# vikasdimaniya/video-fingerprinting

Hardware: AMD Instinct MI355X
Metric: 1080p frames/sec embed+detect (higher is better)
Workload: dtype f32

## Files before the change

### video-fingerprinting_amd/csrc/offmark_kernels.hip

```cpp
#include <hip/hip_runtime.h>
#include <hip/hip_ext.h>

#include <atomic>
#include <cstdint>
#include <cstdio>
#include <cstring>
#include <type_traits>

#include "../../include/offmark_hip.h"

#include "common.hiph"
#include "readout.hiph"
#include "dct_kernels.hiph"
#include "svd_kernels.hiph"
#include "svd8_kernels.hiph"
#include "misc_kernels.hiph"
#include "planar_kernels.hiph"
#include "svd_planar_kernels.hiph"
#include "copies_kernels.hiph"
#include "planar_copies_kernels.hiph"
#include "resync_kernels.hiph"
#include "dct_resync_kernels.hiph"
#include "planar_resync_kernels.hiph"

// ... 77 lines not shown
    const unsigned grid = (unsigned)(vec < 256 * 2048 ? (vec + 255) / 256 : 2048);
    hipLaunchKernelGGL(zero_kernel, dim3(grid), dim3(256), 0, s, static_cast<uint8_t *>(p), bytes);
    return hipGetLastError();
}

constexpr int kMaxChunk = 65535;

template <class Body>
int for_chunks(int n, int cap, Body &&body) {
    for (int f0 = 0; f0 < n; f0 += cap)
        if (int rc = body(f0, n - f0 < cap ? n - f0 : cap)) return rc;
    return OFMK_OK;
}

template <class F>
void with_bool(bool b, F &&f) {
    if (b) f(std::true_type{});
    else f(std::false_type{});
}
template <class F>
void with_fmt(int layout, F &&f) {
    if (layout == OFMK_YUV_I420) f(std::integral_constant<int, FMT_I420>{});
    else f(std::integral_constant<int, FMT_NV12>{});
}
template <class F>
void with_svd_mode(int mode, bool multi, F &&f) {
    if (mode == SVD_DETECT) f(std::integral_constant<int, SVD_DETECT>{}, std::false_type{});
    else if (mode == SVD_DETECT_SOFT) f(std::integral_constant<int, SVD_DETECT_SOFT>{}, std::false_type{});
    else if (mode == SVD_EMBED) with_bool(multi, [&](auto mu) { f(std::integral_constant<int, SVD_EMBED>{}, mu); });
    else with_bool(multi, [&](auto mu) { f(std::integral_constant<int, SVD_EMBED_VERIFY>{}, mu); });
}

struct Workspace {
    float *rec;
    float *delta;
    unsigned long long *ysum;
    unsigned long long *ysum2;
    int frames;
    int tiles;
    size_t plane;
};

constexpr size_t kFixedBytes = 4096;

size_t tiles_per_frame(int H, int W) { return ((size_t)(H / 8) * (W / 8) + kThreads - 1) / kThreads; }

size_t per_frame_bytes(int H, int W) {
    const size_t nblk = (size_t)(H / 8) * (W / 8);
    return nblk * (kRec + 1) * sizeof(float) + 2 * tiles_per_frame(H, W) * 8;
}

int carve(void *ws, size_t bytes, int H, int W, int want_frames, Workspace &out) {
    if (!ws) return fail(OFMK_E_ARG, "workspace is null%s");
    if ((uintptr_t)ws % 256) return fail(OFMK_E_ARG, "workspace must be 256-byte aligned%s");
    const size_t per = per_frame_bytes(H, W);
    if (bytes < per + kFixedBytes) return fail(OFMK_E_WORKSPACE, "workspace smaller than ofmk_workspace_bytes(1, H, W)%s");
    size_t cap = (bytes - kFixedBytes) / per;
    if (want_frames > 0 && (size_t)want_frames < cap) cap = want_frames;
    if (cap > (size_t)kMaxChunk) cap = kMaxChunk;
    const size_t nblk = (size_t)(H / 8) * (W / 8);
    char *p = static_cast<char *>(ws);
    out.frames = (int)cap;
    out.tiles = (int)tiles_per_frame(H, W);
    out.plane = cap * nblk;
    out.rec = reinterpret_cast<float *>(p);
    p += align256(out.plane * kRec * sizeof(float));
    out.delta = reinterpret_cast<float *>(p);
    p += align256(out.plane * sizeof(float));
    out.ysum = reinterpret_cast<unsigned long long *>(p);
    p += align256(cap * out.tiles * 8);
    out.ysum2 = reinterpret_cast<unsigned long long *>(p);
    return OFMK_OK;
}

int check_opts(const ofmk_opts *o) {
    if (o && ((o->flags & ~(uint32_t)(OFMK_F_SEPARATE_DETECT | OFMK_F_LINEAR_TILES | OFMK_F_XCD_TILES | OFMK_F_PARTIAL_COUNTS)) || o->xcds > 64u))
        return fail(OFMK_E_ARG, "ofmk_opts: unknown flag bits or xcds > 64%s");
    if (o && (o->flags & OFMK_F_LINEAR_TILES) && (o->flags & OFMK_F_XCD_TILES))
        return fail(OFMK_E_ARG, "ofmk_opts: OFMK_F_LINEAR_TILES and OFMK_F_XCD_TILES exclude each other%s");
    return OFMK_OK;
}

int check_dims(int n, int H, int W) {
    if (n <= 0) return fail(OFMK_E_ARG, "n must be positive%s");
    if (H < 8 || W < 8) return fail(OFMK_E_ARG, "H and W must be at least 8%s");
    if ((long long)H * W >= (1LL << 28)) return fail(OFMK_E_ARG, "frame too large (H*W must be < 2^28)%s");
    return OFMK_OK;
}

int check_embed_args(const void *in, const void *out, int n, int H, int W, const uint8_t *wm, int n_wm) {
    int rc = check_dims(n, H, W);
    if (rc) return rc;
    if (!in || !out || !wm) return fail(OFMK_E_ARG, "null frame or watermark pointer%s");
    if (n_wm < 1) return fail(OFMK_E_ARG, "n_wm must be >= 1%s");
    return OFMK_OK;
}

int check_detect_args(const void *in, int n, int H, int W, int L, const int32_t *counts, const uint8_t *bits) {
    int rc = check_dims(n, H, W);
    if (rc) return rc;
    if (!in) return fail(OFMK_E_ARG, "null frame pointer%s");
    if (L < 1) return fail(OFMK_E_ARG, "payload length L must be >= 1%s");
    if (!counts && !bits) return fail(OFMK_E_ARG, "both outputs (counts, bits) are null%s");
    return OFMK_OK;
}

int check_soft_args(const void *in, int n, int H, int W, int L, const long long *soft) {
    if (int rc = check_dims(n, H, W)) return rc;
    if (!in || !soft) return fail(OFMK_E_ARG, "null pointer%s");
    if (L < 1) return fail(OFMK_E_ARG, "payload length L must be >= 1%s");
    return OFMK_OK;
}

Geom make_geom(int H, int W, const Workspace &ws, int frames = 0, int xcds = 0) {
    Geom g;
    g.frames = frames;
    g.xcds = xcds;
    g.W = W;
    g.wb = W / 8;
    g.inv_wb = 1.0f / (float)g.wb;
    g.nblk = (H / 8) * (W / 8);
    g.frame_stride = (size_t)H * W * 3;
    g.plane = ws.plane;
    return g;
}

dim3 grid_2d(int units_per_frame, int n) { return dim3((unsigned)((units_per_frame + kThreads - 1) / kThreads), (unsigned)n); }

dim3 xcd_grid(int blocks_per_frame, int n, int xcds = 0) {
    const unsigned tiles = (unsigned)((blocks_per_frame + kThreads - 1) / kThreads);
    const unsigned long long G = (unsigned long long)tiles * (unsigned)n;
    const unsigned long long X = xcds > 1 ? (unsigned long long)xcds : 1ull;
    return dim3((unsigned)(((G + X - 1) / X) * X));
}

bool aligned_rows(const void *p, int W, size_t elem) {
    const size_t need = elem == 1 ? 8 : 16;
    return W % 8 == 0 && (uintptr_t)p % need == 0;
}

void launch_copy_fringe(const uint8_t *in, uint8_t *out, int n, int H, int W, int Hc, int Wc, hipStream_t s) {
    const size_t fringe = (size_t)(H - Hc) * W * 3 + (size_t)Hc * (W - Wc) * 3;
    if (fringe == 0) return;
    const unsigned gx = (unsigned)((fringe + 256 * 4 - 1) / (256 * 4));
    for_chunks(n, kMaxChunk, [&](int f0, int cf) {
        const size_t fo = (size_t)f0 * H * W * 3;
        hipLaunchKernelGGL(copy_fringe_kernel, dim3(gx < 1024 ? gx : 1024, (unsigned)cf), dim3(256), 0, s, in + fo, out + fo, H, W, Hc, Wc);
        return OFMK_OK;
    });
}

int launch_copy_fringe_copies(const uint8_t *in, uint8_t *out, int copies, int n, int H, int W, hipStream_t s) {
    if (H % 8 == 0 && W % 8 == 0) return OFMK_OK;
    for (int q = 0; q < copies; ++q) launch_copy_fringe(in, out + (size_t)q * n * H * W * 3, n, H, W, (H / 8) * 8, (W / 8) * 8, s);
    HIP_TRY(hipGetLastError());
    return OFMK_OK;
}

int launch_analyze(const void *frames, int src, int n, int H, int W, const Workspace &ws, const Ctx &cx,
                   int32_t *zero_counts = nullptr, int L = 0) {
    hipStream_t s = cx.s;
    const Geom g = make_geom(H, W, ws, n);
    const dim3 grid = xcd_grid(g.nblk, n);
    ScopedTiming timing(KIND_ANALYZE, cx);
    constexpr unsigned kAnalyzeLdsCap = 48u * 1024u;
    with_bool(aligned_rows(frames, W, src == SRC_RGB8 ? 1 : 4), [&](auto al) {
        constexpr bool AL = decltype(al)::value;
        if (src == SRC_RGB8) OFMK_TIMED_LAUNCH(timing, (analyze_kernel<SRC_RGB8, AL>), grid, dim3(kThreads), kAnalyzeLdsCap, s, frames, g, ws.rec, ws.ysum, zero_counts, L);
        else OFMK_TIMED_LAUNCH(timing, (analyze_kernel<SRC_YUV32F, AL>), grid, dim3(kThreads), 0, s, frames, g, ws.rec, ws.ysum, zero_counts, L);
    });
    HIP_TRY(hipGetLastError());
    return OFMK_OK;
}

int launch_finalize(FinArgs a, int n, const Ctx &cx) {
    const int per_wg = kThreads * kFinItems;
    const dim3 grid((unsigned)((a.N + per_wg - 1) / per_wg), (unsigned)n);
    ScopedTiming timing(KIND_FINALIZE, cx);
    with_bool(a.delta || a.soft || a.y_dc || a.lum || a.tex || a.step || a.c21_pre || a.c21_post, [&](auto full) {
        OFMK_TIMED_LAUNCH(timing, finalize_kernel<decltype(full)::value>, grid, dim3(kThreads), 0, cx.s, a);
    });
    HIP_TRY(hipGetLastError());
    return OFMK_OK;
}

MarkArgs mark_args(const Workspace &ws, int H, int W, const uint8_t *wm, int n_wm, const int32_t *wm_row, double alpha) {
    MarkArgs m;
    m.rec = ws.rec;
    m.ysum = ws.ysum;
    m.wm = wm;
    m.wm_row = wm_row;
    m.n_wm = n_wm;
    m.N = (int)((long long)H * W / 64);
    m.alpha = alpha;
    return m;
}

int launch_mark_rgb8(const uint8_t *in, uint8_t *out, int n, int H, int W, const uint8_t *wm, int n_wm, const int32_t *wm_row,
                     double alpha, const Workspace &ws, bool fused, const Ctx &cx) {
    hipStream_t s = cx.s;
    const int xc = tile_xcds(cx, (size_t)n * H * W * 3);
    const Geom g = make_geom(H, W, ws, n, xc);
    const dim3 grid = xcd_grid(g.nblk, n, xc);
    const MarkArgs m = mark_args(ws, H, W, wm, n_wm, wm_row, alpha);
    {
        ScopedTiming timing(fused ? KIND_MARK_FUSED : KIND_MARK, cx);
        with_bool(aligned_rows(in, W, 1) && aligned_rows(out, W, 1), [&](auto al) {
            constexpr bool AL = decltype(al)::value;
            if (fused) OFMK_TIMED_LAUNCH(timing, (mark_rgb8_kernel<AL, true>), grid, dim3(kThreads), 0, s, in, out, g, m, ws.rec, ws.ysum2);
            else if (xc > 1) OFMK_TIMED_LAUNCH(timing, (mark_rgb8_kernel<AL, false, true>), grid, dim3(kThreads), 0, s, in, out, g, m, ws.rec, ws.ysum2);
            else OFMK_TIMED_LAUNCH(timing, (mark_rgb8_kernel<AL, false>), grid, dim3(kThreads), 0, s, in, out, g, m, ws.rec, ws.ysum2);
        });
    }
    HIP_TRY(hipGetLastError());
    if (in != out && (H % 8 || W % 8)) {
        launch_copy_fringe(in, out, n, H, W, (H / 8) * 8, (W / 8) * 8, s);
        HIP_TRY(hipGetLastError());
    }
    return OFMK_OK;
}

struct RecView {
    const float *rec;
    const unsigned long long *ysum;
    size_t plane;
    int tiles;
};
RecView input_records(const Workspace &ws) { return {ws.rec, ws.ysum, ws.plane, ws.tiles}; }
RecView marked_records(const Workspace &ws) { return {ws.rec, ws.ysum2, ws.plane, ws.tiles}; }

FinArgs fin_base(const RecView &v, int H, int W, double alpha) {
    FinArgs a;
    memset(&a, 0, sizeof(a));
    a.rec = v.rec;
    a.plane = v.plane;
    a.ysum = v.ysum;
    a.tiles = v.tiles;
    a.nblk = (H / 8) * (W / 8);
    a.N = (int)((long long)H * W / 64);
    a.L = 1;
    a.n_wm = 1;
    a.alpha = alpha;
    return a;
}

int launch_mark_yuv32f(float *yuv, int n, int H, int W, const uint8_t *wm, int n_wm, const int32_t *wm_row, double alpha,
                       const Workspace &ws, const Ctx &cx) {
    FinArgs a = fin_base(input_records(ws), H, W, alpha);
    a.wm = wm;
    a.wm_row = wm_row;
    a.n_wm = n_wm;
    a.delta = ws.delta;
    if (int rc = launch_finalize(a, n, cx)) return rc;
    const Geom g = make_geom(H, W, ws);
    hipLaunchKernelGGL(mark_yuv32f_kernel, grid_2d(g.nblk, n), dim3(kThreads), 0, cx.s, yuv, g, ws.delta);
    HIP_TRY(hipGetLastError());
    return OFMK_OK;
}

int launch_payloads(const int32_t *counts, int n, int L, int n_bits, const int32_t *perm, uint8_t *payload, hipStream_t s) {
    hipLaunchKernelGGL(degenerate_kernel, dim3((unsigned)n), dim3(kThreads), 0, s, counts, L, n_bits, perm, payload);
    HIP_TRY(hipGetLastError());
    return OFMK_OK;
}

CopyArgs make_copy_args(int copies, int n, int f0, const int32_t *wm_rows, size_t frame_bytes, size_t counts_per_frame = 0,
                        size_t bits_per_frame = 0) {
    CopyArgs k;
    memset(&k, 0, sizeof(k));
    k.copies = copies;
    k.rows_stride = n;
    k.wm_rows = wm_rows ? wm_rows + f0 : nullptr;
    k.out_stride = (size_t)n * frame_bytes;
    k.counts_stride = (size_t)n * counts_per_frame;
    k.bits_stride = (size_t)n * bits_per_frame;
    return k;
}

int launch_mark_copies_rgb8(const uint8_t *in, uint8_t *out, int copies, int n, int f0, int cf, int H, int W, const uint8_t *wm,
                            int n_wm, const int32_t *wm_rows, double alpha, const Workspace &ws, const Ctx &cx) {
    const size_t fs = (size_t)H * W * 3;
    const uint8_t *pin = in + (size_t)f0 * fs;
    uint8_t *pout = out + (size_t)f0 * fs;
    const int xc = tile_xcds(cx, (size_t)cf * fs);
    const Geom g = make_geom(H, W, ws, cf, xc);
    const dim3 grid = xcd_grid(g.nblk, cf, xc);
    const MarkArgs m = mark_args(ws, H, W, wm, n_wm, nullptr, alpha);
    const CopyArgs k = make_copy_args(copies, n, f0, wm_rows, fs);
    ScopedTiming timing(KIND_MARK, cx);
    with_bool(aligned_rows(in, W, 1) && aligned_rows(out, W, 1), [&](auto al) {
        OFMK_TIMED_LAUNCH(timing, mark_copies_rgb8_kernel<decltype(al)::value>, grid, dim3(kThreads), 0, cx.s, pin, pout, g, m, k);
    });
    HIP_TRY(hipGetLastError());
    return OFMK_OK;
}

struct CopiesWorkspace {
    Workspace base;
    float *rec;
    unsigned long long *ysum;
    size_t plane;
};

size_t per_frame_copies_bytes(int copies, int H, int W) {
    const size_t nblk = (size_t)(H / 8) * (W / 8);
    return per_frame_bytes(H, W) + (size_t)copies * (nblk * kRec * sizeof(float) + tiles_per_frame(H, W) * 8);
}

int carve_copies(void *ws, size_t bytes, int copies, int H, int W, int want_frames, CopiesWorkspace &out) {
    if (!ws) return fail(OFMK_E_ARG, "workspace is null%s");
    if ((uintptr_t)ws % 256) return fail(OFMK_E_ARG, "workspace must be 256-byte aligned%s");
    const size_t per = per_frame_copies_bytes(copies, H, W);
    if (bytes < per + kFixedBytes) return fail(OFMK_E_WORKSPACE, "workspace smaller than ofmk_copies_workspace_bytes(1, copies, H, W)%s");
    size_t cap = (bytes - kFixedBytes) / per;
    if (want_frames > 0 && (size_t)want_frames < cap) cap = want_frames;
    if (cap > (size_t)kMaxChunk) cap = kMaxChunk;
    if (int rc = carve(ws, bytes, H, W, (int)cap, out.base)) return rc;
    const size_t nblk = (size_t)(H / 8) * (W / 8);
    char *p = reinterpret_cast<char *>(out.base.ysum2) + align256(cap * out.base.tiles * 8);
    out.plane = (size_t)copies * cap * nblk;
    out.rec = reinterpret_cast<float *>(p);
    p += align256(out.plane * kRec * sizeof(float));
    out.ysum = reinterpret_cast<unsigned long long *>(p);
    return OFMK_OK;
}

RecView copy_records(const CopiesWorkspace &ws, int q, int nblk) {
    return {ws.rec + (size_t)q * ws.base.frames * nblk, ws.ysum + (size_t)q * ws.base.frames * ws.base.tiles, ws.plane, ws.base.tiles};
}

int launch_mark_verify_copies_rgb8(const uint8_t *in, uint8_t *out, int copies, int n, int f0, int cf, int H, int W, const uint8_t *wm,
                                   int n_wm, const int32_t *wm_rows, double alpha, int L, const CopyRecs &v, const Workspace &ws,
                                   const Ctx &cx) {
    const size_t fs = (size_t)H * W * 3;
    const uint8_t *pin = in + (size_t)f0 * fs;
    uint8_t *pout = out + (size_t)f0 * fs;
    const int xc = tile_xcds(cx, (size_t)cf * fs);
    const Geom g = make_geom(H, W, ws, cf, xc);
    const dim3 grid = xcd_grid(g.nblk, cf, xc);
    const MarkArgs m = mark_args(ws, H, W, wm, n_wm, nullptr, alpha);
    const CopyArgs k = make_copy_args(copies, n, f0, wm_rows, fs, (size_t)L, (size_t)m.N);
    ScopedTiming timing(KIND_MARK_FUSED, cx);
    with_bool(aligned_rows(in, W, 1) && aligned_rows(out, W, 1), [&](auto al) {
        OFMK_TIMED_LAUNCH(timing, mark_verify_copies_rgb8_kernel<decltype(al)::value>, grid, dim3(kThreads), 0, cx.s, pin, pout, g, m, k, v);
    });
    HIP_TRY(hipGetLastError());
    return OFMK_OK;
}

int check_planar(int layout, int H, int W, const void *a, const void *b) {
    if (layout != OFMK_YUV_I420 && layout != OFMK_YUV_NV12) return fail(OFMK_E_ARG, "layout must be OFMK_YUV_I420 or OFMK_YUV_NV12%s");
    if (H % 8 || W % 8) return fail(OFMK_E_ARG, "planar 4:2:0 entry points need H and W to be multiples of 8%s");
    if ((a && (uintptr_t)a % 8) || (b && (uintptr_t)b % 8)) return fail(OFMK_E_ARG, "planar frame buffers must be 8-byte aligned%s");
    return OFMK_OK;
}

PGeom make_pgeom(int layout, int H, int W, size_t plane) {
    PGeom g;
    g.W = W;
    g.wb = W / 8;
    g.inv_wb = 1.0f / (float)g.wb;
    g.nblk = (H / 8) * (W / 8);
    g.frame_stride = (size_t)H * W * 3 / 2;
    g.u_off = (size_t)H * W;
    g.v_off = layout == OFMK_YUV_I420 ? g.u_off + (size_t)H * W / 4 : g.u_off + 1;
    g.cpitch = layout == OFMK_YUV_I420 ? W / 2 : W;
    g.plane = plane;
    return g;
}

int launch_analyze_yuv420(const uint8_t *frames, int layout, int n, int H, int W, const Workspace &ws, const Ctx &cx,
                          int32_t *zero_counts = nullptr, int L = 0) {
    const PGeom g = make_pgeom(layout, H, W, ws.plane);
    ScopedTiming timing(KIND_PLANAR_ANALYZE, cx);
    with_fmt(layout, [&](auto fmt) {
        OFMK_TIMED_LAUNCH(timing, analyze_yuv420_kernel<decltype(fmt)::value>, grid_2d(g.nblk, n), dim3(kThreads), 0, cx.s, frames, g, ws.rec, ws.ysum, zero_counts, L);
    });
    HIP_TRY(hipGetLastError());
    return OFMK_OK;
}

int launch_mark_yuv420(const uint8_t *in, uint8_t *out, int layout, int n, int H, int W, const uint8_t *wm, int n_wm, const int32_t *wm_row,
                       double alpha, const Workspace &ws, bool fused, const Ctx &cx) {
    const PGeom g = make_pgeom(layout, H, W, ws.plane);
    const MarkArgs m = mark_args(ws, H, W, wm, n_wm, wm_row, alpha);
    ScopedTiming timing(KIND_PLANAR_MARK, cx);
    with_fmt(layout, [&](auto fmt) { with_bool(fused, [&](auto fu) {
        OFMK_TIMED_LAUNCH(timing, (mark_yuv420_kernel<decltype(fmt)::value, decltype(fu)::value>), grid_2d(g.nblk, n), dim3(kThreads), 0, cx.s, in, out, g, m, ws.rec, ws.ysum2);
    }); });
    HIP_TRY(hipGetLastError());
    return OFMK_OK;
}

int convert_yuv420(uint8_t *yuv, uint8_t *rgb, bool to_rgb, int layout, int n, int H, int W, void *stream, const ofmk_opts *opts) {
    if (int orc = check_opts(opts)) return orc;
    int rc = check_dims(n, H, W);
    if (rc) return rc;
    if (!yuv || !rgb) return fail(OFMK_E_ARG, "null pointer%s");
    if ((rc = check_planar(layout, H, W, yuv, rgb))) return rc;
    const PGeom g = make_pgeom(layout, H, W, 0);
    hipStream_t s = static_cast<hipStream_t>(stream);
    for_chunks(n, kMaxChunk, [&](int f0, int cf) {
        uint8_t *py = yuv + (size_t)f0 * g.frame_stride, *pr = rgb + (size_t)f0 * H * W * 3;
        with_fmt(layout, [&](auto fmt) {
            if (to_rgb) hipLaunchKernelGGL(yuv420_to_rgb8_kernel<decltype(fmt)::value>, grid_2d(g.nblk, cf), dim3(kThreads), 0, s, py, pr, g);
            else hipLaunchKernelGGL(rgb8_to_yuv420_kernel<decltype(fmt)::value>, grid_2d(g.nblk, cf), dim3(kThreads), 0, s, pr, py, g);
        });
        return OFMK_OK;
    });
    HIP_TRY(hipGetLastError());
    return OFMK_OK;
}

Geom8 make_geom8(int H, int W) {
    Geom8 g;
    g.W = W;
    g.wt = ((W / 4) * 2) / 8;
    g.inv_wt = g.wt ? 1.0f / (float)g.wt : 0.f;
    g.ntile = (((H / 4) * 2) / 8) * g.wt;
    g.frames = 0;
    g.frame_stride = (size_t)H * W * 3;
    return g;
}

Geom svd_geom(int H, int W) {
    Workspace none;
    none.plane = 0;
    return make_geom(H, W, none);
}

int svd_count_tiles(int H, int W, int blk) {
    const long long units = blk == 8 ? (long long)make_geom8(H, W).ntile : (long long)(H / 8) * (W / 8);
    return (int)((units + kThreads - 1) / kThreads);
}

int check_partial(const ofmk_opts *o, int L, const int32_t *counts, int &partial) {
    partial = (o && (o->flags & OFMK_F_PARTIAL_COUNTS)) ? 1 : 0;
    if (partial && !counts) return fail(OFMK_E_ARG, "OFMK_F_PARTIAL_COUNTS without a counts buffer%s");
    if (partial && L > kHistMax) return fail(OFMK_E_ARG, "OFMK_F_PARTIAL_COUNTS needs L <= 2048 (longer payloads: plain counts)%s");
    return OFMK_OK;
}

int check_blk(int blk) {
    if (blk != 4 && blk != 8)
        return fail(OFMK_E_ARG, "blk must be 4 (the reference's default) or 8%s");
    return OFMK_OK;
}

int set_scales(SvdArgs &a, const double *scales, bool need_channel1) {
    if (!scales) return fail(OFMK_E_ARG, "scales is null (host array of 3 doubles)%s");
    bool any = false;
    for (int k = 0; k < 3; ++k) {
        if (!(scales[k] == scales[k]) || scales[k] > 1e30 || scales[k] < -1e30) return fail(OFMK_E_ARG, "scales must be finite%s");
        const float sc = scales[k] > 0 ? (float)scales[k] : 0.f;
        if (scales[k] > 0 && !(sc >= 1.0e-3f)) return fail(OFMK_E_ARG, "a positive scale must be >= 1e-3 as float32%s");
        a.scales[k] = sc;
        any |= sc > 0.f;
    }
    if (!any && !need_channel1) return fail(OFMK_E_ARG, "no channel has a positive scale%s");
    return OFMK_OK;
}

// ... 75 lines not shown
        const Geom8 g = make_geom8(H, W);
        const int N8 = (int)((long long)H * W / 256);
        Hc = (((H / 4) * 2) / 8) * 16, Wc = g.wt * 16;
        const bool al = W % 8 == 0 && (uintptr_t)in % 8 == 0 && (reads || (uintptr_t)out % 8 == 0);
        rc = launch_svd({g.ntile, N8, g.frame_stride, 1, cw}, n, a, cx, [&](SvdChunk &c) {
            Geom8 gc = g;
            gc.frames = c.frames;
            with_bool(al, [&](auto al_) { with_svd_mode(mode, c.multi, [&](auto md, auto mu) {
                OFMK_TIMED_LAUNCH(c.timing, (svd8_rgb8_kernel<decltype(al_)::value, decltype(md)::value, decltype(mu)::value>), c.grid, dim3(kThreads), 0, cx.s,
                                  in + c.offset, out ? out + c.offset : nullptr, gc, to_args8(c.a, N8));
            }); });
        });
    } else {
        const Geom g = svd_geom(H, W);
        const bool al = aligned_rows(in, W, 1) && (reads || aligned_rows(out, W, 1));
        rc = launch_svd({g.nblk, a.N, g.frame_stride, 1, cw}, n, a, cx, [&](SvdChunk &c) {
            Geom gc = g;
            gc.frames = c.frames;
            with_bool(al, [&](auto al_) { with_svd_mode(mode, c.multi, [&](auto md, auto mu) {
                OFMK_TIMED_LAUNCH(c.timing, (svd_rgb8_kernel<decltype(al_)::value, decltype(md)::value, decltype(mu)::value>), c.grid, dim3(kThreads), 0, cx.s,
                                  in + c.offset, out ? out + c.offset : nullptr, gc, c.a);
            }); });
        });
    }
    if (rc) return rc;
    if (!reads && in != out && (Hc != H || Wc != W)) {
        launch_copy_fringe(in, out, n, H, W, Hc, Wc, cx.s);
        HIP_TRY(hipGetLastError());
    }
    return OFMK_OK;
}

int launch_svd_yuv420(const uint8_t *in, uint8_t *out, int layout, int n, int H, int W, int mode, int blk, const SvdArgs &a, const Ctx &cx) {
    const PGeom g = make_pgeom(layout, H, W, 0);
    const int cw = mode == SVD_DETECT_SOFT ? 2 : 1;
    if (blk == 4)
        return launch_svd({g.nblk, a.N, g.frame_stride, 1, cw}, n, a, cx, [&](SvdChunk &c) {
            with_fmt(layout, [&](auto fmt) { with_svd_mode(mode, c.multi, [&](auto md, auto mu) {
                OFMK_TIMED_LAUNCH(c.timing, (svd_yuv420_kernel<decltype(fmt)::value, decltype(md)::value, decltype(mu)::value>), c.grid, dim3(kThreads), 0, cx.s,
                                  in + c.offset, out ? out + c.offset : nullptr, g, c.frames, c.a);
            }); });
        });
    const Geom8 g8 = make_geom8(H, W);
    const int N8 = (int)((long long)H * W / 256);
    int rc = launch_svd({g8.ntile, N8, g.frame_stride, 1, cw}, n, a, cx, [&](SvdChunk &c) {
        Geom8 gc = g8;
        gc.frames = c.frames;
        with_fmt(layout, [&](auto fmt) { with_svd_mode(mode, c.multi, [&](auto md, auto mu) {
            OFMK_TIMED_LAUNCH(c.timing, (svd8_yuv420_kernel<decltype(fmt)::value, decltype(md)::value, decltype(mu)::value>), c.grid, dim3(kThreads), 0, cx.s,
                              in + c.offset, out ? out + c.offset : nullptr, g, gc, to_args8(c.a, N8));
        }); });
    });
    if (rc) return rc;
    const int hcb = (((H / 4) * 2) / 8) * 2, wcb = g8.wt * 2;
    const int nfringe = g.nblk - hcb * wcb;
    if (mode == SVD_DETECT || mode == SVD_DETECT_SOFT || nfringe <= 0) return OFMK_OK;
    for_chunks(n, kMaxChunk, [&](int f0, int cf) {
        const size_t fo = (size_t)f0 * g.frame_stride;
        ScopedTiming timing(KIND_SVD, cx);
        with_fmt(layout, [&](auto fmt) {
            OFMK_TIMED_LAUNCH(timing, svd_fringe_yuv420_kernel<decltype(fmt)::value>, grid_2d(nfringe, cf), dim3(kThreads), 0, cx.s, in + fo, out + fo, g, hcb, wcb, nfringe);
        });
        return OFMK_OK;
    });
    HIP_TRY(hipGetLastError());
    return OFMK_OK;
}
// ... 44 lines not shown
    if (o0 < i0 + fb && i0 < o0 + fb * (size_t)copies) return fail(OFMK_E_ARG, "out must not overlap in (no in-place copies)%s");
    return OFMK_OK;
}

int launch_svd_copies_rgb8(const uint8_t *in, uint8_t *out, int copies, int n, int H, int W, const int32_t *wm_rows, const SvdArgs &a,
                           const Ctx &cx, long long *soft = nullptr) {
    const Geom g = svd_geom(H, W);
    const bool verify = a.counts || a.bits;
    const size_t count_rows = a.partial ? (size_t)svd_count_tiles(H, W, 4) : 1;
    const bool al = aligned_rows(in, W, 1) && aligned_rows(out, W, 1);
    int rc = launch_svd({g.nblk, a.N, g.frame_stride, copies}, n, a, cx, [&](SvdChunk &c) {
        const CopyArgs kc = make_copy_args(copies, n, c.f0, wm_rows, g.frame_stride, count_rows * a.L, a.N);
        Geom gc = g;
        gc.frames = c.frames;
        if (soft) {
            const CopySoft sf{soft + (size_t)c.f0 * a.L, (size_t)n * a.L};
            with_bool(al, [&](auto al_) { with_bool(c.multi, [&](auto mu) {
                OFMK_TIMED_LAUNCH(c.timing, (svd_copies_soft_rgb8_kernel<decltype(al_)::value, decltype(mu)::value>), c.grid, dim3(kThreads), 0, cx.s,
                                  in + c.offset, out + c.offset, gc, c.a, kc, sf);
            }); });
            return;
        }
        with_bool(al, [&](auto al_) { with_bool(verify, [&](auto vf) { with_bool(c.multi, [&](auto mu) {
            OFMK_TIMED_LAUNCH(c.timing, (svd_copies_rgb8_kernel<decltype(al_)::value, decltype(vf)::value, decltype(mu)::value>), c.grid, dim3(kThreads), 0, cx.s,
                              in + c.offset, out + c.offset, gc, c.a, kc);
        }); }); });
    });
    if (rc) return rc;
    return launch_copy_fringe_copies(in, out, copies, n, H, W, cx.s);
}

int launch_mark_copies_yuv420(const uint8_t *in, uint8_t *out, int layout, int copies, int n, int f0, int cf, int H, int W,
                              const uint8_t *wm, int n_wm, const int32_t *wm_rows, double alpha, const Workspace &ws, const Ctx &cx) {
    const PGeom g = make_pgeom(layout, H, W, ws.plane);
    const MarkArgs m = mark_args(ws, H, W, wm, n_wm, nullptr, alpha);
    const CopyArgs k = make_copy_args(copies, n, f0, wm_rows, g.frame_stride);
    const size_t fo = (size_t)f0 * g.frame_stride;
    ScopedTiming timing(KIND_PLANAR_MARK, cx);
    with_fmt(layout, [&](auto fmt) {
        OFMK_TIMED_LAUNCH(timing, mark_copies_yuv420_kernel<decltype(fmt)::value>, grid_2d(g.nblk, cf), dim3(kThreads), 0, cx.s, in + fo, out + fo, g, m, k);
    });
    HIP_TRY(hipGetLastError());
    return OFMK_OK;
}

int launch_mark_verify_copies_yuv420(const uint8_t *in, uint8_t *out, int layout, int copies, int n, int f0, int cf, int H, int W,
                                     const uint8_t *wm, int n_wm, const int32_t *wm_rows, double alpha, int L, const CopyRecs &v,
                                     const Workspace &ws, const Ctx &cx) {
    const PGeom g = make_pgeom(layout, H, W, ws.plane);
    const MarkArgs m = mark_args(ws, H, W, wm, n_wm, nullptr, alpha);
    const CopyArgs k = make_copy_args(copies, n, f0, wm_rows, g.frame_stride, (size_t)L, (size_t)m.N);
    const dim3 grid = grid_2d(g.nblk, cf);
    if ((int)grid.x != ws.tiles) return fail(OFMK_E_ARG, "internal: tile count of the launch and of the workspace differ%s");
    const size_t fo = (size_t)f0 * g.frame_stride;
    ScopedTiming timing(KIND_PLANAR_MARK, cx);
    with_fmt(layout, [&](auto fmt) {
        OFMK_TIMED_LAUNCH(timing, mark_verify_copies_yuv420_kernel<decltype(fmt)::value>, grid, dim3(kThreads), 0, cx.s, in + fo, out + fo, g, m, k, v);
    });
    HIP_TRY(hipGetLastError());
    return OFMK_OK;
}

int launch_svd_copies_yuv420(const uint8_t *in, uint8_t *out, int layout, int copies, int n, int H, int W, const int32_t *wm_rows,
                             const SvdArgs &a, const Ctx &cx, long long *soft = nullptr) {
    const PGeom g = make_pgeom(layout, H, W, 0);
    const bool verify = a.counts || a.bits;
    const size_t count_rows = a.partial ? (size_t)svd_count_tiles(H, W, 4) : 1;
    return launch_svd({g.nblk, a.N, g.frame_stride, copies}, n, a, cx, [&](SvdChunk &c) {
        const CopyArgs kc = make_copy_args(copies, n, c.f0, wm_rows, g.frame_stride, count_rows * a.L, a.N);
        if (soft) {
            const CopySoft sf{soft + (size_t)c.f0 * a.L, (size_t)n * a.L};
            with_fmt(layout, [&](auto fmt) { with_bool(c.multi, [&](auto mu) {
                OFMK_TIMED_LAUNCH(c.timing, (svd_copies_soft_yuv420_kernel<decltype(fmt)::value, decltype(mu)::value>), c.grid, dim3(kThreads), 0, cx.s,
                                  in + c.offset, out + c.offset, g, c.frames, c.a, kc, sf);
            }); });
            return;
        }
        with_fmt(layout, [&](auto fmt) { with_bool(verify, [&](auto vf) { with_bool(c.multi, [&](auto mu) {
            OFMK_TIMED_LAUNCH(c.timing, (svd_copies_yuv420_kernel<decltype(fmt)::value, decltype(vf)::value, decltype(mu)::value>), c.grid, dim3(kThreads), 0, cx.s,
                              in + c.offset, out + c.offset, g, c.frames, c.a, kc);
        }); }); });
    });
}

template <class Fused, class Single, class SoftOf>
int svd_copies_soft(uint8_t *out, size_t frame_bytes, int copies, int n, int H, int W, int blk, int L, const int32_t *wm_rows, SvdArgs a,
                    long long *soft, const Ctx &cx, Fused &&fused, Single &&single, SoftOf &&soft_of) {
    a.L = L;
    HIP_TRY(launch_zero(soft, (size_t)copies * n * L * sizeof(long long), cx.s));
    const bool on = a.scales[1] > 0.f;
    if (blk == 4) return fused(a, on ? soft : nullptr);
    return launch_svd8_copies(out, frame_bytes, copies, n, H, W, wm_rows, a, [&](uint8_t *out_q, const SvdArgs &b) {
        if (int rc = single(out_q, b)) return rc;
        if (!on) return (int)OFMK_OK;
        const size_t q = (size_t)(out_q - out) / ((size_t)n * frame_bytes);
        SvdArgs bs = b;
        bs.counts = reinterpret_cast<int32_t *>(soft + q * n * L);
        bs.bits = nullptr;
// ... 11 lines not shown
};
FrameFmt rgb8_frames(int H, int W) { return {FRAMES_RGB8, 0, H, W, (size_t)H * W * 3}; }
FrameFmt yuv32f_frames(int H, int W) { return {FRAMES_YUV32F, 0, H, W, (size_t)H * W * 3 * sizeof(float)}; }
FrameFmt yuv420_frames(int layout, int H, int W) { return {FRAMES_YUV420, layout, H, W, (size_t)H * W * 3 / 2}; }

int analyze_frames(const FrameFmt &f, const uint8_t *frames, int n, const Workspace &ws, const Ctx &cx, int32_t *zero_counts = nullptr,
                   int L = 0) {
    if (f.kind == FRAMES_YUV420) return launch_analyze_yuv420(frames, f.layout, n, f.H, f.W, ws, cx, zero_counts, L);
    return launch_analyze(frames, f.kind == FRAMES_RGB8 ? SRC_RGB8 : SRC_YUV32F, n, f.H, f.W, ws, cx, zero_counts, L);
}

int mark_frames(const FrameFmt &f, const uint8_t *in, uint8_t *out, int n, const uint8_t *wm, int n_wm, const int32_t *wm_row,
                double alpha, const Workspace &ws, bool fused, const Ctx &cx) {
    if (f.kind == FRAMES_RGB8) return launch_mark_rgb8(in, out, n, f.H, f.W, wm, n_wm, wm_row, alpha, ws, fused, cx);
    if (f.kind == FRAMES_YUV420) return launch_mark_yuv420(in, out, f.layout, n, f.H, f.W, wm, n_wm, wm_row, alpha, ws, fused, cx);
    if (fused || in != out) return fail(OFMK_E_ARG, "internal: float32 frames are marked in place, without verify%s");
    return launch_mark_yuv32f(reinterpret_cast<float *>(out), n, f.H, f.W, wm, n_wm, wm_row, alpha, ws, cx);
}

int mark_copies(const FrameFmt &f, const uint8_t *in, uint8_t *out, int copies, int n, int f0, int cf, const uint8_t *wm, int n_wm,
                const int32_t *wm_rows, double alpha, const Workspace &ws, const Ctx &cx) {
    if (f.kind == FRAMES_RGB8) return launch_mark_copies_rgb8(in, out, copies, n, f0, cf, f.H, f.W, wm, n_wm, wm_rows, alpha, ws, cx);
    if (f.kind == FRAMES_YUV420)
        return launch_mark_copies_yuv420(in, out, f.layout, copies, n, f0, cf, f.H, f.W, wm, n_wm, wm_rows, alpha, ws, cx);
    return fail(OFMK_E_ARG, "internal: no copies kernel for float32 frames%s");
}

int mark_verify_copies(const FrameFmt &f, const uint8_t *in, uint8_t *out, int copies, int n, int f0, int cf, const uint8_t *wm,
                       int n_wm, const int32_t *wm_rows, double alpha, int L, int32_t *zero_counts, const CopiesWorkspace &ws,
                       const Ctx &cx) {
    CopyRecs v;
    v.rec = ws.rec;
    v.ysum = ws.ysum;
    v.plane = ws.plane;
    v.rec_stride = (size_t)ws.base.frames * (f.H / 8) * (f.W / 8);
    v.ysum_stride = (size_t)ws.base.frames * ws.base.tiles;
    v.zero_counts = zero_counts ? zero_counts + (size_t)f0 * L : nullptr;
    v.L = L;
    if (f.kind == FRAMES_RGB8)
        return launch_mark_verify_copies_rgb8(in, out, copies, n, f0, cf, f.H, f.W, wm, n_wm, wm_rows, alpha, L, v, ws.base, cx);
    if (f.kind == FRAMES_YUV420)
        return launch_mark_verify_copies_yuv420(in, out, f.layout, copies, n, f0, cf, f.H, f.W, wm, n_wm, wm_rows, alpha, L, v, ws.base, cx);
    return fail(OFMK_E_ARG, "internal: no copies kernel for float32 frames%s");
}

int read_out(const RecView &v, const FrameFmt &f, size_t row, int cf, int L, double alpha, int32_t *counts, uint8_t *bits,
             long long *soft, const Ctx &cx) {
    FinArgs a = fin_base(v, f.H, f.W, alpha);
    a.L = L;
    if (counts || bits) {
        a.counts = counts ? counts + row * L : nullptr;
        a.bits = bits ? bits + row * a.N : nullptr;
        if (int rc = launch_finalize(a, cf, cx)) return rc;
    }
    if (!soft) return OFMK_OK;
    a.counts = nullptr;
    a.bits = nullptr;
    a.soft = soft + row * L;
    return launch_finalize(a, cf, cx);
}

int embed_chunk(const FrameFmt &f, const uint8_t *in, uint8_t *out, int f0, int cf, const uint8_t *wm, int n_wm, const int32_t *wm_row,
                double alpha, const Workspace &ws, bool verify, const Ctx &cx, int32_t *zero_counts = nullptr, int L = 0) {
    const size_t fo = (size_t)f0 * f.frame_bytes;
    if (int rc = analyze_frames(f, in + fo, cf, ws, cx, zero_counts ? zero_counts + (size_t)f0 * L : nullptr, L)) return rc;
    return mark_frames(f, in + fo, out + fo, cf, wm, n_wm, wm_row ? wm_row + f0 : nullptr, alpha, ws, verify, cx);
}
// ... 55 lines not shown
                               const int32_t *wm_rows, double alpha, int L, int32_t *counts, uint8_t *bits, long long *soft,
                               int chunk_frames, void *workspace, size_t workspace_bytes, void *stream, const ofmk_opts *opts) {
    CopiesWorkspace ws;
    if (int rc = carve_copies(workspace, workspace_bytes, copies, f.H, f.W, chunk_frames, ws)) return rc;
    const Ctx cx = make_ctx(stream, opts);
    const bool hard = counts || bits;
    const int nblk = (f.H / 8) * (f.W / 8);
    const size_t N = (size_t)((long long)f.H * f.W / 64);
    if (soft) HIP_TRY(launch_zero(soft, (size_t)copies * n * L * sizeof(long long), cx.s));
    int rc = for_chunks(n, ws.base.frames, [&](int f0, int cf) {
        if (int rc = analyze_frames(f, in + (size_t)f0 * f.frame_bytes, cf, ws.base, cx)) return rc;
        if (!(cx.flags & OFMK_F_SEPARATE_DETECT)) {
            if (int rc = mark_verify_copies(f, in, out, copies, n, f0, cf, wm, n_wm, wm_rows, alpha, L, counts, ws, cx)) return rc;
            for (int q = 0; q < copies; ++q)
                if (int rc = read_out(copy_records(ws, q, nblk), f, (size_t)q * n + f0, cf, L, alpha, counts, bits, soft, cx)) return rc;
            return (int)OFMK_OK;
        }
        if (int rc = mark_copies(f, in, out, copies, n, f0, cf, wm, n_wm, wm_rows, alpha, ws.base, cx)) return rc;
        for (int q = 0; q < copies; ++q) {
            const uint8_t *out_q = out + (size_t)q * n * f.frame_bytes;
            if (hard)
                if (int rc = detect_chunk(f, out_q, f0, cf, L, alpha, counts ? counts + (size_t)q * n * L : nullptr,
                                          bits ? bits + (size_t)q * n * N : nullptr, nullptr, ws.base, cx)) return rc;
            if (soft)
                if (int rc = detect_chunk(f, out_q, f0, cf, L, alpha, nullptr, nullptr, soft + (size_t)q * n * L, ws.base, cx)) return rc;
        }
        return (int)OFMK_OK;
    });
    if (rc) return rc;
    return launch_copy_fringe_copies(in, out, copies, n, f.H, f.W, cx.s);
}

struct SyncWorkspace {
    float *rec;
    unsigned long long *sums;
    int frames;
    size_t norig;
};
size_t sync_per_frame_bytes(int H, int W) { return (size_t)(H - 7) * (W - 7) * kRec * sizeof(float) + 64 * sizeof(unsigned long long); }

int carve_sync(void *ws, size_t bytes, int H, int W, int want_frames, SyncWorkspace &out) {
    if (!ws) return fail(OFMK_E_ARG, "workspace is null%s");
    if ((uintptr_t)ws % 256) return fail(OFMK_E_ARG, "workspace must be 256-byte aligned%s");
    const size_t per = sync_per_frame_bytes(H, W);
    if (bytes < per + kFixedBytes) return fail(OFMK_E_WORKSPACE, "workspace smaller than ofmk_sync_workspace_bytes(1, H, W)%s");
    size_t cap = (bytes - kFixedBytes) / per;
    if (want_frames > 0 && (size_t)want_frames < cap) cap = want_frames;
    if (cap > (size_t)kMaxChunk) cap = kMaxChunk;
    out.frames = (int)cap;
    out.norig = (size_t)(H - 7) * (W - 7);
    out.rec = static_cast<float *>(ws);
    out.sums = reinterpret_cast<unsigned long long *>(static_cast<char *>(ws) + align256(cap * out.norig * kRec * sizeof(float)));
    return OFMK_OK;
}

int check_alpha(double alpha) {
    if (!(alpha > 0.0) || !(alpha <= 1.79769313486231570815e308)) return fail(OFMK_E_ARG, "alpha must be a positive finite number%s");
    return OFMK_OK;
}

int sync_scores_chunk(const uint8_t *in, int f0, int cf, int H, int W, double alpha, long long *scores, const SyncWorkspace &ws,
                      const Ctx &cx) {
    DctSyncGeom g;
    g.H = H;
    g.W = W;
    g.ow = W - 7;
    g.rects_x = (W - 7 + kDsRect * kDsStrip - 1) / (kDsRect * kDsStrip);
    g.frame_stride = (size_t)H * W * 3;
    g.norig = ws.norig;
    g.plane = (size_t)ws.frames * ws.norig;
    const dim3 grid((unsigned)(g.rects_x * ((H - 7 + kDsRect - 1) / kDsRect)), (unsigned)cf);
    HIP_TRY(launch_zero(ws.sums, (size_t)cf * 64 * sizeof(unsigned long long), cx.s));
    {
        ScopedTiming timing(KIND_ANALYZE, cx);
        OFMK_TIMED_LAUNCH(timing, dct_sync_analyze_rgb8_kernel, grid, dim3(kThreads), 0, cx.s, in + (size_t)f0 * g.frame_stride, g, ws.rec,
                          ws.sums);
    }
    {
        ScopedTiming timing(KIND_FINALIZE, cx);
        OFMK_TIMED_LAUNCH(timing, dct_sync_scores_kernel, grid, dim3(kThreads), 0, cx.s, g, ws.rec, ws.sums, alpha,
                          reinterpret_cast<unsigned long long *>(scores) + (size_t)f0 * 64);
    }
    HIP_TRY(hipGetLastError());
    return OFMK_OK;
}

int soft_window_chunk(const uint8_t *in, int f0, int cf, int H, int W, int py, int px, int rows, int cols, int canvas_cols, int base,
                      int L, double alpha, long long *soft, const Workspace &ws, const Ctx &cx) {
    Geom g = make_geom(8 * rows, 8 * cols, ws, cf);
    g.W = W;
    g.frame_stride = (size_t)H * W * 3;
    const uint8_t *first = in + (size_t)f0 * g.frame_stride + ((size_t)py * W + px) * 3;
    {
        ScopedTiming timing(KIND_ANALYZE, cx);
        OFMK_TIMED_LAUNCH(timing, (analyze_kernel<SRC_RGB8, false>), xcd_grid(g.nblk, cf), dim3(kThreads), 0, cx.s,
                          static_cast<const void *>(first), g, ws.rec, ws.ysum, static_cast<int32_t *>(nullptr), 0);
    }
    DctWindowArgs a;
    a.rec = ws.rec;
    a.plane = ws.plane;
    a.ysum = ws.ysum;
    a.tiles = ws.tiles;
    a.nblk = g.nblk;
    a.cols = cols;
    a.canvas_cols = canvas_cols;
    a.base = base;
    a.L = L;
    a.alpha = alpha;
    a.soft = soft + (size_t)f0 * L;
    {
        const int per_wg = kThreads * kFinItems;
        ScopedTiming timing(KIND_FINALIZE, cx);
        OFMK_TIMED_LAUNCH(timing, finalize_soft_window_kernel, dim3((unsigned)((a.nblk + per_wg - 1) / per_wg), (unsigned)cf), dim3(kThreads),
                          0, cx.s, a);
    }
    HIP_TRY(hipGetLastError());
    return OFMK_OK;
}

int check_planar_resync(int layout, int H, int W) {
    if (layout != OFMK_YUV_I420 && layout != OFMK_YUV_NV12) return fail(OFMK_E_ARG, "layout must be OFMK_YUV_I420 or OFMK_YUV_NV12%s");
    if (H % 2 || W % 2) return fail(OFMK_E_ARG, "4:2:0 planes need even H and W%s");
    return OFMK_OK;
}

int check_planar_window(int H, int W, int py, int px, int canvas_cols, int base, int &rows, int &cols) {
    if (py < 0 || py > 7 || px < 0 || px > 7) return fail(OFMK_E_ARG, "the phase (py, px) must be in 0..7%s");
    if (py % 2 || px % 2) return fail(OFMK_E_ARG, "an odd phase does not exist on 4:2:0 planes: py and px must be even%s");
    rows = (H - py) / 8;
    cols = (W - px) / 8;
    if (rows < 1 || cols < 1) return fail(OFMK_E_ARG, "no full 8x8 unit at this phase%s");
    if (canvas_cols < cols) return fail(OFMK_E_ARG, "canvas_cols is smaller than the window's units per row%s");
    if (base < 0) return fail(OFMK_E_ARG, "base must not be negative%s");
// ... 6 lines not shown
    p.H = H;
    p.W = W;
    p.cpitch = layout == OFMK_YUV_I420 ? W / 2 : W;
    p.cstep = layout == OFMK_YUV_I420 ? 1 : 2;
    p.frame_stride = (size_t)H * W * 3 / 2;
    p.u_off = (size_t)H * W;
    p.v_off = layout == OFMK_YUV_I420 ? p.u_off + (size_t)H * W / 4 : p.u_off + 1;
    return p;
}

PWinGeom make_window_geom(int layout, int H, int W, int rows, int cols, int frames) {
    PWinGeom g;
    g.p = make_plane_geom(layout, H, W);
    g.wb = cols;
    g.nblk = rows * cols;
    g.inv_wb = 1.0f / (float)cols;
    g.frames = frames;
    return g;
}

size_t psync_origins(int H, int W) { return (size_t)(H / 2 - 3) * (W / 2 - 3); }
size_t psync_per_frame_bytes(int H, int W) { return psync_origins(H, W) * kRec * sizeof(float) + 16 * sizeof(unsigned long long); }

int carve_psync(void *ws, size_t bytes, int H, int W, int want_frames, SyncWorkspace &out) {
    if (!ws) return fail(OFMK_E_ARG, "workspace is null%s");
    if ((uintptr_t)ws % 256) return fail(OFMK_E_ARG, "workspace must be 256-byte aligned%s");
    const size_t per = psync_per_frame_bytes(H, W);
    if (bytes < per + kFixedBytes) return fail(OFMK_E_WORKSPACE, "workspace smaller than ofmk_sync_workspace_bytes_yuv420(1, H, W)%s");
    size_t cap = (bytes - kFixedBytes) / per;
    if (want_frames > 0 && (size_t)want_frames < cap) cap = want_frames;
    if (cap > (size_t)kMaxChunk) cap = kMaxChunk;
    out.frames = (int)cap;
    out.norig = psync_origins(H, W);
    out.rec = static_cast<float *>(ws);
    out.sums = reinterpret_cast<unsigned long long *>(static_cast<char *>(ws) + align256(cap * out.norig * kRec * sizeof(float)));
    return OFMK_OK;
}

int psync_scores_chunk(const uint8_t *in, int layout, int f0, int cf, int H, int W, double alpha, long long *scores,
                       const SyncWorkspace &ws, const Ctx &cx) {
    PDctSyncGeom g;
    g.p = make_plane_geom(layout, H, W);
    g.oh = H / 2 - 3;
    g.ow = W / 2 - 3;
    g.rects_x = (g.ow + kPdRectX * kPdStrip - 1) / (kPdRectX * kPdStrip);
    g.norig = ws.norig;
    g.plane = (size_t)ws.frames * ws.norig;
    const dim3 grid((unsigned)(g.rects_x * ((g.oh + kPdRectY - 1) / kPdRectY)), (unsigned)cf);
    HIP_TRY(launch_zero(ws.sums, (size_t)cf * 16 * sizeof(unsigned long long), cx.s));
    {
        ScopedTiming timing(KIND_PLANAR_ANALYZE, cx);
        OFMK_TIMED_LAUNCH(timing, dct_sync_analyze_yuv420_kernel, grid, dim3(kThreads), 0, cx.s, in + (size_t)f0 * g.p.frame_stride, g,
                          ws.rec, ws.sums);
    }
    {
        ScopedTiming timing(KIND_FINALIZE, cx);
        OFMK_TIMED_LAUNCH(timing, dct_sync_scores_yuv420_kernel, grid, dim3(kThreads), 0, cx.s, g, ws.rec, ws.sums, alpha,
                          reinterpret_cast<unsigned long long *>(scores) + (size_t)f0 * 64);
    }
    HIP_TRY(hipGetLastError());
    return OFMK_OK;
}

int psoft_window_chunk(const uint8_t *in, int layout, int f0, int cf, int H, int W, int py, int px, int rows, int cols, int canvas_cols,
                       int base, int L, double alpha, long long *soft, const Workspace &ws, const Ctx &cx) {
    const PWinGeom g = make_window_geom(layout, H, W, rows, cols, cf);
    const dim3 grid = grid_2d(g.nblk, cf);
    if ((int)grid.x != ws.tiles) return fail(OFMK_E_ARG, "internal: tile count of the launch and of the workspace differ%s");
    {
        ScopedTiming timing(KIND_PLANAR_ANALYZE, cx);
        OFMK_TIMED_LAUNCH(timing, analyze_window_yuv420_kernel, grid, dim3(kThreads), 0, cx.s, in + (size_t)f0 * g.p.frame_stride, g, py, px,
                          ws.plane, ws.rec, ws.ysum);
    }
    DctWindowArgs a;
    a.rec = ws.rec;
    a.plane = ws.plane;
    a.ysum = ws.ysum;
    a.tiles = ws.tiles;
    a.nblk = g.nblk;
    a.cols = cols;
    a.canvas_cols = canvas_cols;
    a.base = base;
    a.L = L;
    a.alpha = alpha;
    a.soft = soft + (size_t)f0 * L;
    {
        const int per_wg = kThreads * kFinItems;
        ScopedTiming timing(KIND_FINALIZE, cx);
        OFMK_TIMED_LAUNCH(timing, finalize_soft_window_kernel, dim3((unsigned)((a.nblk + per_wg - 1) / per_wg), (unsigned)cf), dim3(kThreads),
                          0, cx.s, a);
    }
    HIP_TRY(hipGetLastError());
    return OFMK_OK;
}

}

extern "C" {

int ofmk_version(void) { return OFMK_ABI_VERSION; }
const char *ofmk_last_error(void) { return g_err; }

size_t ofmk_workspace_bytes(int frames_in_flight, int H, int W) {
    if (frames_in_flight < 1 || H < 8 || W < 8) return 0;
    return per_frame_bytes(H, W) * (size_t)frames_in_flight + kFixedBytes;
}

int ofmk_embed_rgb8(const uint8_t *in, uint8_t *out, int n, int H, int W, const uint8_t *wm, int n_wm,
                    const int32_t *wm_row, double alpha, int chunk_frames, void *workspace, size_t workspace_bytes,
// ... 767 lines not shown
```

Baseline: 282,800.

## Store per-block records as interleaved BlockRec structs instead of planar arrays

Replaces the structure-of-arrays record workspace (kRec float planes with a plane stride) with an array of BlockRec structs, and removes the plane stride from the geometry and argument structs. Each block's record fields become contiguous, so a thread can read or write one record with wide vector accesses instead of kRec strided loads. The cost is that accesses are no longer coalesced across threads for a single field. Only the host side is shown; the kernels in the headers must change to match.

```diff
diff --git a/video-fingerprinting_amd/csrc/offmark_kernels.hip b/video-fingerprinting_amd/csrc/offmark_kernels.hip
--- a/video-fingerprinting_amd/csrc/offmark_kernels.hip
+++ b/video-fingerprinting_amd/csrc/offmark_kernels.hip
@@ -133,13 +133,12 @@
 }
 
 struct Workspace {
-    float *rec;
+    BlockRec *rec;
     float *delta;
     unsigned long long *ysum;
     unsigned long long *ysum2;
     int frames;
     int tiles;
-    size_t plane;
 };
 
 constexpr size_t kFixedBytes = 4096;
@@ -163,11 +162,10 @@
     char *p = static_cast<char *>(ws);
     out.frames = (int)cap;
     out.tiles = (int)tiles_per_frame(H, W);
-    out.plane = cap * nblk;
-    out.rec = reinterpret_cast<float *>(p);
-    p += align256(out.plane * kRec * sizeof(float));
+    out.rec = reinterpret_cast<BlockRec *>(p);
+    p += align256(cap * nblk * sizeof(BlockRec));
     out.delta = reinterpret_cast<float *>(p);
-    p += align256(out.plane * sizeof(float));
+    p += align256(cap * nblk * sizeof(float));
     out.ysum = reinterpret_cast<unsigned long long *>(p);
     p += align256(cap * out.tiles * 8);
     out.ysum2 = reinterpret_cast<unsigned long long *>(p);
@@ -213,7 +211,7 @@
     return OFMK_OK;
 }
 
-Geom make_geom(int H, int W, const Workspace &ws, int frames = 0, int xcds = 0) {
+Geom make_geom(int H, int W, int frames = 0, int xcds = 0) {
     Geom g;
     g.frames = frames;
     g.xcds = xcds;
@@ -222,7 +220,6 @@
     g.inv_wb = 1.0f / (float)g.wb;
     g.nblk = (H / 8) * (W / 8);
     g.frame_stride = (size_t)H * W * 3;
-    g.plane = ws.plane;
     return g;
 }
 
@@ -261,7 +258,7 @@
 int launch_analyze(const void *frames, int src, int n, int H, int W, const Workspace &ws, const Ctx &cx,
                    int32_t *zero_counts = nullptr, int L = 0) {
     hipStream_t s = cx.s;
-    const Geom g = make_geom(H, W, ws, n);
+    const Geom g = make_geom(H, W, n);
     const dim3 grid = xcd_grid(g.nblk, n);
     ScopedTiming timing(KIND_ANALYZE, cx);
     constexpr unsigned kAnalyzeLdsCap = 48u * 1024u;
@@ -301,7 +298,7 @@
                      double alpha, const Workspace &ws, bool fused, const Ctx &cx) {
     hipStream_t s = cx.s;
     const int xc = tile_xcds(cx, (size_t)n * H * W * 3);
-    const Geom g = make_geom(H, W, ws, n, xc);
+    const Geom g = make_geom(H, W, n, xc);
     const dim3 grid = xcd_grid(g.nblk, n, xc);
     const MarkArgs m = mark_args(ws, H, W, wm, n_wm, wm_row, alpha);
     {
@@ -322,19 +319,17 @@
 }
 
 struct RecView {
-    const float *rec;
+    const BlockRec *rec;
     const unsigned long long *ysum;
-    size_t plane;
     int tiles;
 };
-RecView input_records(const Workspace &ws) { return {ws.rec, ws.ysum, ws.plane, ws.tiles}; }
-RecView marked_records(const Workspace &ws) { return {ws.rec, ws.ysum2, ws.plane, ws.tiles}; }
+RecView input_records(const Workspace &ws) { return {ws.rec, ws.ysum, ws.tiles}; }
+RecView marked_records(const Workspace &ws) { return {ws.rec, ws.ysum2, ws.tiles}; }
 
 FinArgs fin_base(const RecView &v, int H, int W, double alpha) {
     FinArgs a;
     memset(&a, 0, sizeof(a));
     a.rec = v.rec;
-    a.plane = v.plane;
     a.ysum = v.ysum;
     a.tiles = v.tiles;
     a.nblk = (H / 8) * (W / 8);
@@ -353,7 +348,7 @@
     a.n_wm = n_wm;
     a.delta = ws.delta;
     if (int rc = launch_finalize(a, n, cx)) return rc;
-    const Geom g = make_geom(H, W, ws);
+    const Geom g = make_geom(H, W);
     hipLaunchKernelGGL(mark_yuv32f_kernel, grid_2d(g.nblk, n), dim3(kThreads), 0, cx.s, yuv, g, ws.delta);
     HIP_TRY(hipGetLastError());
     return OFMK_OK;
@@ -384,7 +379,7 @@
     const uint8_t *pin = in + (size_t)f0 * fs;
     uint8_t *pout = out + (size_t)f0 * fs;
     const int xc = tile_xcds(cx, (size_t)cf * fs);
-    const Geom g = make_geom(H, W, ws, cf, xc);
+    const Geom g = make_geom(H, W, cf, xc);
     const dim3 grid = xcd_grid(g.nblk, cf, xc);
     const MarkArgs m = mark_args(ws, H, W, wm, n_wm, nullptr, alpha);
     const CopyArgs k = make_copy_args(copies, n, f0, wm_rows, fs);
@@ -398,9 +393,8 @@
 
 struct CopiesWorkspace {
     Workspace base;
-    float *rec;
+    BlockRec *rec;
     unsigned long long *ysum;
-    size_t plane;
 };
 
 size_t per_frame_copies_bytes(int copies, int H, int W) {
@@ -419,15 +413,14 @@
     if (int rc = carve(ws, bytes, H, W, (int)cap, out.base)) return rc;
     const size_t nblk = (size_t)(H / 8) * (W / 8);
     char *p = reinterpret_cast<char *>(out.base.ysum2) + align256(cap * out.base.tiles * 8);
-    out.plane = (size_t)copies * cap * nblk;
-    out.rec = reinterpret_cast<float *>(p);
-    p += align256(out.plane * kRec * sizeof(float));
+    out.rec = reinterpret_cast<BlockRec *>(p);
+    p += align256((size_t)copies * cap * nblk * sizeof(BlockRec));
     out.ysum = reinterpret_cast<unsigned long long *>(p);
     return OFMK_OK;
 }
 
 RecView copy_records(const CopiesWorkspace &ws, int q, int nblk) {
-    return {ws.rec + (size_t)q * ws.base.frames * nblk, ws.ysum + (size_t)q * ws.base.frames * ws.base.tiles, ws.plane, ws.base.tiles};
+    return {ws.rec + (size_t)q * ws.base.frames * nblk, ws.ysum + (size_t)q * ws.base.frames * ws.base.tiles, ws.base.tiles};
 }
 
 int launch_mark_verify_copies_rgb8(const uint8_t *in, uint8_t *out, int copies, int n, int f0, int cf, int H, int W, const uint8_t *wm,
@@ -437,7 +430,7 @@
     const uint8_t *pin = in + (size_t)f0 * fs;
     uint8_t *pout = out + (size_t)f0 * fs;
     const int xc = tile_xcds(cx, (size_t)cf * fs);
-    const Geom g = make_geom(H, W, ws, cf, xc);
+    const Geom g = make_geom(H, W, cf, xc);
     const dim3 grid = xcd_grid(g.nblk, cf, xc);
     const MarkArgs m = mark_args(ws, H, W, wm, n_wm, nullptr, alpha);
     const CopyArgs k = make_copy_args(copies, n, f0, wm_rows, fs, (size_t)L, (size_t)m.N);
@@ -456,7 +449,7 @@
     return OFMK_OK;
 }
 
-PGeom make_pgeom(int layout, int H, int W, size_t plane) {
+PGeom make_pgeom(int layout, int H, int W) {
     PGeom g;
     g.W = W;
     g.wb = W / 8;
@@ -466,13 +459,12 @@
     g.u_off = (size_t)H * W;
     g.v_off = layout == OFMK_YUV_I420 ? g.u_off + (size_t)H * W / 4 : g.u_off + 1;
     g.cpitch = layout == OFMK_YUV_I420 ? W / 2 : W;
-    g.plane = plane;
     return g;
 }
 
 int launch_analyze_yuv420(const uint8_t *frames, int layout, int n, int H, int W, const Workspace &ws, const Ctx &cx,
                           int32_t *zero_counts = nullptr, int L = 0) {
-    const PGeom g = make_pgeom(layout, H, W, ws.plane);
+    const PGeom g = make_pgeom(layout, H, W);
     ScopedTiming timing(KIND_PLANAR_ANALYZE, cx);
     with_fmt(layout, [&](auto fmt) {
         OFMK_TIMED_LAUNCH(timing, analyze_yuv420_kernel<decltype(fmt)::value>, grid_2d(g.nblk, n), dim3(kThreads), 0, cx.s, frames, g, ws.rec, ws.ysum, zero_counts, L);
@@ -483,7 +475,7 @@
 
 int launch_mark_yuv420(const uint8_t *in, uint8_t *out, int layout, int n, int H, int W, const uint8_t *wm, int n_wm, const int32_t *wm_row,
                        double alpha, const Workspace &ws, bool fused, const Ctx &cx) {
-    const PGeom g = make_pgeom(layout, H, W, ws.plane);
+    const PGeom g = make_pgeom(layout, H, W);
     const MarkArgs m = mark_args(ws, H, W, wm, n_wm, wm_row, alpha);
     ScopedTiming timing(KIND_PLANAR_MARK, cx);
     with_fmt(layout, [&](auto fmt) { with_bool(fused, [&](auto fu) {
@@ -499,7 +491,7 @@
     if (rc) return rc;
     if (!yuv || !rgb) return fail(OFMK_E_ARG, "null pointer%s");
     if ((rc = check_planar(layout, H, W, yuv, rgb))) return rc;
-    const PGeom g = make_pgeom(layout, H, W, 0);
+    const PGeom g = make_pgeom(layout, H, W);
     hipStream_t s = static_cast<hipStream_t>(stream);
     for_chunks(n, kMaxChunk, [&](int f0, int cf) {
         uint8_t *py = yuv + (size_t)f0 * g.frame_stride, *pr = rgb + (size_t)f0 * H * W * 3;
@@ -524,11 +516,7 @@
     return g;
 }
 
-Geom svd_geom(int H, int W) {
-    Workspace none;
-    none.plane = 0;
-    return make_geom(H, W, none);
-}
+Geom svd_geom(int H, int W) { return make_geom(H, W); }
 
 int svd_count_tiles(int H, int W, int blk) {
     const long long units = blk == 8 ? (long long)make_geom8(H, W).ntile : (long long)(H / 8) * (W / 8);
@@ -670,7 +658,7 @@
 }
 
 int launch_svd_yuv420(const uint8_t *in, uint8_t *out, int layout, int n, int H, int W, int mode, int blk, const SvdArgs &a, const Ctx &cx) {
-    const PGeom g = make_pgeom(layout, H, W, 0);
+    const PGeom g = make_pgeom(layout, H, W);
     const int cw = mode == SVD_DETECT_SOFT ? 2 : 1;
     if (blk == 4)
         return launch_svd({g.nblk, a.N, g.frame_stride, 1, cw}, n, a, cx, [&](SvdChunk &c) {
@@ -781,7 +769,7 @@
 
 int launch_mark_copies_yuv420(const uint8_t *in, uint8_t *out, int layout, int copies, int n, int f0, int cf, int H, int W,
                               const uint8_t *wm, int n_wm, const int32_t *wm_rows, double alpha, const Workspace &ws, const Ctx &cx) {
-    const PGeom g = make_pgeom(layout, H, W, ws.plane);
+    const PGeom g = make_pgeom(layout, H, W);
     const MarkArgs m = mark_args(ws, H, W, wm, n_wm, nullptr, alpha);
     const CopyArgs k = make_copy_args(copies, n, f0, wm_rows, g.frame_stride);
     const size_t fo = (size_t)f0 * g.frame_stride;
@@ -796,7 +784,7 @@
 int launch_mark_verify_copies_yuv420(const uint8_t *in, uint8_t *out, int layout, int copies, int n, int f0, int cf, int H, int W,
                                      const uint8_t *wm, int n_wm, const int32_t *wm_rows, double alpha, int L, const CopyRecs &v,
                                      const Workspace &ws, const Ctx &cx) {
-    const PGeom g = make_pgeom(layout, H, W, ws.plane);
+    const PGeom g = make_pgeom(layout, H, W);
     const MarkArgs m = mark_args(ws, H, W, wm, n_wm, nullptr, alpha);
     const CopyArgs k = make_copy_args(copies, n, f0, wm_rows, g.frame_stride, (size_t)L, (size_t)m.N);
     const dim3 grid = grid_2d(g.nblk, cf);
@@ -812,7 +800,7 @@
 
 int launch_svd_copies_yuv420(const uint8_t *in, uint8_t *out, int layout, int copies, int n, int H, int W, const int32_t *wm_rows,
                              const SvdArgs &a, const Ctx &cx, long long *soft = nullptr) {
-    const PGeom g = make_pgeom(layout, H, W, 0);
+    const PGeom g = make_pgeom(layout, H, W);
     const bool verify = a.counts || a.bits;
     const size_t count_rows = a.partial ? (size_t)svd_count_tiles(H, W, 4) : 1;
     return launch_svd({g.nblk, a.N, g.frame_stride, copies}, n, a, cx, [&](SvdChunk &c) {
@@ -890,7 +878,6 @@
     CopyRecs v;
     v.rec = ws.rec;
     v.ysum = ws.ysum;
-    v.plane = ws.plane;
     v.rec_stride = (size_t)ws.base.frames * (f.H / 8) * (f.W / 8);
     v.ysum_stride = (size_t)ws.base.frames * ws.base.tiles;
     v.zero_counts = zero_counts ? zero_counts + (size_t)f0 * L : nullptr;
@@ -1012,7 +999,7 @@
 }
 
 struct SyncWorkspace {
-    float *rec;
+    BlockRec *rec;
     unsigned long long *sums;
     int frames;
     size_t norig;
@@ -1029,7 +1016,7 @@
     if (cap > (size_t)kMaxChunk) cap = kMaxChunk;
     out.frames = (int)cap;
     out.norig = (size_t)(H - 7) * (W - 7);
-    out.rec = static_cast<float *>(ws);
+    out.rec = static_cast<BlockRec *>(ws);
     out.sums = reinterpret_cast<unsigned long long *>(static_cast<char *>(ws) + align256(cap * out.norig * kRec * sizeof(float)));
     return OFMK_OK;
 }
@@ -1048,7 +1035,6 @@
     g.rects_x = (W - 7 + kDsRect * kDsStrip - 1) / (kDsRect * kDsStrip);
     g.frame_stride = (size_t)H * W * 3;
     g.norig = ws.norig;
-    g.plane = (size_t)ws.frames * ws.norig;
     const dim3 grid((unsigned)(g.rects_x * ((H - 7 + kDsRect - 1) / kDsRect)), (unsigned)cf);
     HIP_TRY(launch_zero(ws.sums, (size_t)cf * 64 * sizeof(unsigned long long), cx.s));
     {
@@ -1067,7 +1053,7 @@
 
 int soft_window_chunk(const uint8_t *in, int f0, int cf, int H, int W, int py, int px, int rows, int cols, int canvas_cols, int base,
                       int L, double alpha, long long *soft, const Workspace &ws, const Ctx &cx) {
-    Geom g = make_geom(8 * rows, 8 * cols, ws, cf);
+    Geom g = make_geom(8 * rows, 8 * cols, cf);
     g.W = W;
     g.frame_stride = (size_t)H * W * 3;
     const uint8_t *first = in + (size_t)f0 * g.frame_stride + ((size_t)py * W + px) * 3;
@@ -1078,7 +1064,6 @@
     }
     DctWindowArgs a;
     a.rec = ws.rec;
-    a.plane = ws.plane;
     a.ysum = ws.ysum;
     a.tiles = ws.tiles;
     a.nblk = g.nblk;
@@ -1151,7 +1136,7 @@
     if (cap > (size_t)kMaxChunk) cap = kMaxChunk;
     out.frames = (int)cap;
     out.norig = psync_origins(H, W);
-    out.rec = static_cast<float *>(ws);
+    out.rec = static_cast<BlockRec *>(ws);
     out.sums = reinterpret_cast<unsigned long long *>(static_cast<char *>(ws) + align256(cap * out.norig * kRec * sizeof(float)));
     return OFMK_OK;
 }
@@ -1164,7 +1149,6 @@
     g.ow = W / 2 - 3;
     g.rects_x = (g.ow + kPdRectX * kPdStrip - 1) / (kPdRectX * kPdStrip);
     g.norig = ws.norig;
-    g.plane = (size_t)ws.frames * ws.norig;
     const dim3 grid((unsigned)(g.rects_x * ((g.oh + kPdRectY - 1) / kPdRectY)), (unsigned)cf);
     HIP_TRY(launch_zero(ws.sums, (size_t)cf * 16 * sizeof(unsigned long long), cx.s));
     {
@@ -1189,11 +1173,10 @@
     {
         ScopedTiming timing(KIND_PLANAR_ANALYZE, cx);
         OFMK_TIMED_LAUNCH(timing, analyze_window_yuv420_kernel, grid, dim3(kThreads), 0, cx.s, in + (size_t)f0 * g.p.frame_stride, g, py, px,
-                          ws.plane, ws.rec, ws.ysum);
+                          ws.rec, ws.ysum);
     }
     DctWindowArgs a;
     a.rec = ws.rec;
-    a.plane = ws.plane;
     a.ysum = ws.ysum;
     a.tiles = ws.tiles;
     a.nblk = g.nblk;
```

Result: no change. 282,400 (-0.1%).
